# NickDrake117/GNNkeras

Hardware: AMD Instinct MI355X
Metric: node-state updates/s (arcs x iterations / s), forward Loop (higher is better)
Workload: dtype f32; 1 GPU; C4 Erdos-Renyi 1000000 nodes / 10000000 arcs, state_dim=64, max_iteration=50, threshold=0 (k=50), node-focused, average aggregation, BN+Dense(159->64,selu) state net

## Files before the change

gnnkeras_amd/csrc/kernels_train_big.hpp:

```cpp
#pragma once
#include "bf16_split.hpp"
#include <hip/hip_runtime.h>
#include "kernels_general.hpp"
#include "kernel_state_fused4.hpp"
#include <type_traits>
#include "kernel_state_lds.hpp"
#include "kernels_train.hpp"
#include "buffer_ops.hpp"

namespace gnn {

constexpr int TB_STREAM_AUX = 0;
constexpr int TB_RING_AUX = 2;
#define TB_MFMA_DRAIN() asm volatile("s_nop 15\n\ts_nop 3" ::: "memory")
typedef float f32x16 __attribute__((ext_vector_type(16)));
constexpr int TB_WAVES = 8;

template <int LPR, bool HAS_W, bool BUF = false>
__global__ void __launch_bounds__(256, 8)
k_aggregate_stats(const int *gate, int n_dst, const int *__restrict__ rowptr, const int *__restrict__ src,
                  const float *__restrict__ w, const float *__restrict__ row_scale, const float *__restrict__ X, int ldx,
                  float *__restrict__ out, int ldo, float *__restrict__ stat_part, const float *__restrict__ shift) {
    if (gate_closed(gate)) return;
    __shared__ f32x4 red[2][256];
// ... 174 lines not shown
    return activate1<ACT>(v);
}
__device__ __forceinline__ f32x4 fma4(const f32x4 &a, const f32x4 &b, const f32x4 &c) { return __builtin_elementwise_fma(a, b, c); }

__device__ __forceinline__ void split3_store(unsigned short *base, int plane_stride, int idx, float v) {
    const __bf16 vh = (__bf16)v;
    const float r1 = v - (float)vh;
    const __bf16 vm = (__bf16)r1;
    const float r2 = r1 - (float)vm;
    const __bf16 vl = (__bf16)r2;
    base[idx] = __builtin_bit_cast(unsigned short, vh); base[plane_stride + idx] = __builtin_bit_cast(unsigned short, vm);
    base[2 * plane_stride + idx] = __builtin_bit_cast(unsigned short, vl);
}


constexpr int TB_B6_WAVES = 2;
template <int SQ, int ACT, bool ADD>
__device__ __forceinline__ void train_fwd_b6_body(const TrainFwdArgs &a, const int bid, const int nblk) {
    if (gate_closed(a.gate)) return;
    constexpr int XQ = ADD ? 0 : 2;
    constexpr int NCT = SQ, HP = 16 * NCT, NQ = 2 * SQ + XQ, NKB = NQ / 2;
    constexpr int PLANE = NKB * NCT * 64 * 8;
    extern __shared__ __attribute__((aligned(16))) float tb_smem[];
    unsigned short *Wl = reinterpret_cast<unsigned short *>(tb_smem);
    float *bias_l = tb_smem + 3 * PLANE / 2;
    float *red = bias_l + HP;
    float *shift_l = red + TB_WAVES * 2 * HP;
    float *mean_l = shift_l + HP;
    __shared__ int any_s;
    const int tid = threadIdx.x, lane = tid & 63, wave = tid >> 6;
    const int c = lane & 15, g = lane >> 4;
    if (tid == 0) any_s = 0;
    for (int h = tid; h < HP; h += 64 * TB_WAVES) shift_l[h] = (a.stat_shift && h < a.H) ? a.stat_shift[h] : 0.0f;
    for (int k = tid; k < 16 * NQ; k += 64 * TB_WAVES) mean_l[k] = fwd_in_mean(a, SQ, k);
    int *rowtab = reinterpret_cast<int *>(red);
    for (int k = tid; k < 16 * NQ; k += 64 * TB_WAVES) {
        int row = -1;
        if (k < 16 * SQ) row = a.wrow_state + k;
        else if (k < 32 * SQ) row = a.wrow_agg + (k - 16 * SQ);
        else if (!ADD && a.xc) {
            int jj = k - 32 * SQ, beg = 0;
#pragma unroll
            for (int sg = 0; sg < 3; ++sg) {
                if (sg < a.cs.n && jj >= beg && jj < beg + a.cs.width[sg]) row = a.cs.wrow[sg] + (jj - beg);
                if (sg < a.cs.n) beg += a.cs.width[sg];
            }
        }
        rowtab[k] = row;
    }
    __syncthreads();
    {
        const __amdgpu_buffer_rsrc_t r_w = buf_rsrc(a.Wf);
        constexpr int PER = (16 * NQ * HP) / (64 * TB_WAVES), BATCH = PER % 5 == 0 ? 5 : PER % 4 == 0 ? 4 : PER % 3 == 0 ? 3 : PER % 2 == 0 ? 2 : 1;
        static_assert((16 * NQ * HP) % (64 * TB_WAVES) == 0 && (64 * TB_WAVES) % HP == 0 && PER % BATCH == 0, "weight staging: whole batches");
        const int h = tid % HP, k0 = tid / HP;
#pragma unroll 1
        for (int it0 = 0; it0 < PER; it0 += BATCH) {
            float v[BATCH];
#pragma unroll
            for (int u = 0; u < BATCH; ++u) {
                const int k = k0 + (it0 + u) * ((64 * TB_WAVES) / HP), row = rowtab[k];
                v[u] = buf_ld_f32(r_w, (row >= 0 && h < a.H) ? ((unsigned)row * (unsigned)a.H + (unsigned)h) * 4u : BUF_OFF);
            }
#pragma unroll
            for (int u = 0; u < BATCH; ++u) {
                const int k = k0 + (it0 + u) * ((64 * TB_WAVES) / HP);
                const int q = k >> 4, gg = (k >> 2) & 3, e = k & 3;
                split3_store(Wl, PLANE, ((((q >> 1) * NCT + (h >> 4)) * 64 + 16 * gg + (h & 15)) * 8) + 4 * (q & 1) + e, v[u]);
            }
        }
    }
    __syncthreads();
    for (int h = tid; h < HP; h += 64 * TB_WAVES) bias_l[h] = h < a.H ? a.bf[h] : 0.0f;
    __syncthreads();

    const __amdgpu_buffer_rsrc_t r_s = buf_rsrc_n(a.state, (unsigned)a.M * (unsigned)a.ld_state * 4u), r_a = buf_rsrc_n(a.agg, (unsigned)a.M * (unsigned)a.ld_agg * 4u),
                                 r_x = ADD ? buf_rsrc_n(uniform_ptr(a.addend), (unsigned)a.M * (unsigned)a.ld_add * 4u) : buf_rsrc_n(uniform_ptr(a.xc), (unsigned)a.M * 128u),
                                 r_y = buf_rsrc(a.Y);
    const int n_tiles = (a.M + 15) >> 4;
    f32x4 cs1[NCT], cs2[NCT];
#pragma unroll
    for (int ct = 0; ct < NCT; ++ct) { cs1[ct] = (f32x4){0.f, 0.f, 0.f, 0.f}; cs2[ct] = (f32x4){0.f, 0.f, 0.f, 0.f}; }
    int any = 0;
    f32x4 A[NQ];
    f32x4 Cn[ADD ? NCT : 1];
    const unsigned o_s = (unsigned)c * (unsigned)a.ld_state * 4u + 16u * g, o_a = (unsigned)c * (unsigned)a.ld_agg * 4u + 16u * g,
                   o_x = ADD ? (unsigned)c * (unsigned)a.ld_add * 4u + 16u * g : (unsigned)c * 128u + 16u * g;
    auto fetch = [&](int t) {
        const unsigned b_s = 64u * (unsigned)t * (unsigned)a.ld_state + o_s, b_a = 64u * (unsigned)t * (unsigned)a.ld_agg + o_a,
                       b_x = ADD ? 64u * (unsigned)t * (unsigned)a.ld_add + o_x : 2048u * (unsigned)t + o_x;
#pragma unroll
        for (int q = 0; q < SQ; ++q) {
            A[q] = buf_ld_f32x4_aux<TB_STREAM_AUX>(r_s, b_s + 64u * q);
            A[SQ + q] = buf_ld_f32x4_aux<TB_STREAM_AUX>(r_a, b_a + 64u * q);
        }
        if constexpr (ADD) {
#pragma unroll
            for (int ct = 0; ct < NCT; ++ct) Cn[ct] = buf_ld_f32x4_aux<TB_STREAM_AUX>(r_x, b_x + 64u * ct);
        } else {
#pragma unroll
            for (int q = 0; q < XQ; ++q) A[2 * SQ + q] = buf_ld_f32x4_aux<TB_STREAM_AUX>(r_x, b_x + 64u * q);
        }
    };
    const int t_step = nblk * TB_WAVES;
    fetch(bid * TB_WAVES + wave);
    const u32x4 *Wv = reinterpret_cast<const u32x4 *>(Wl) + lane;
    f32x4 vP[NCT];
    int offP = 0; bool inP = false;
#pragma unroll
    for (int ct = 0; ct < NCT; ++ct) vP[ct] = (f32x4){0.f, 0.f, 0.f, 0.f};
#pragma unroll 1
    for (int t = bid * TB_WAVES + wave; t < n_tiles; t += t_step) {
        const int row = 16 * t + c;
        const bool in = row < a.M;
        u32x4 xh[NKB], xm[NKB], xl[NKB];
        f32x4 old[SQ];
#pragma unroll
        for (int kb = 0; kb < NKB; ++kb)
            split3_x8pk(A[2 * kb] - *reinterpret_cast<const f32x4 *>(mean_l + 32 * kb + 4 * g), A[2 * kb + 1] - *reinterpret_cast<const f32x4 *>(mean_l + 32 * kb + 16 + 4 * g),
                        xh[kb], xm[kb], xl[kb]);
#pragma unroll
        for (int q = 0; q < SQ; ++q) old[q] = A[q];
        f32x4 acc[NCT];
#pragma unroll
        for (int ct = 0; ct < NCT; ++ct) {
            acc[ct] = *reinterpret_cast<const f32x4 *>(bias_l + 16 * ct + 4 * g);
            if constexpr (ADD) acc[ct] += Cn[ct];
        }
        __builtin_amdgcn_sched_barrier(0);
        fetch(t + t_step);
#pragma unroll
        for (int ct = 0; ct < NCT; ++ct) {
            const u32x4 bits = {__float_as_uint(vP[ct][0]), __float_as_uint(vP[ct][1]), __float_as_uint(vP[ct][2]), __float_as_uint(vP[ct][3])};
            __builtin_amdgcn_raw_buffer_store_b128(bits, r_y, inP ? offP + (int)((16u * ct + 4u * g) * 4u) : (int)BUF_OFF, 0, 0);
        }
        __builtin_amdgcn_sched_barrier(0);
        constexpr int CTG = NCT < 2 ? NCT : 2, SPK = NCT / CTG, NS = NKB * SPK;
        u32x4 W[2][3][CTG];
        auto load_w = [&](int st, u32x4 (&w)[3][CTG]) {
            const int kb = st / SPK, ct0 = (st % SPK) * CTG;
#pragma unroll
            for (int pl = 0; pl < 3; ++pl)
#pragma unroll
                for (int u = 0; u < CTG; ++u) w[pl][u] = Wv[pl * (PLANE / 8) + (kb * NCT + ct0 + u) * 64];
        };
        load_w(0, W[0]);
#pragma unroll
        for (int st = 0; st < NS; ++st) {
            const int kb = st / SPK, ct0 = (st % SPK) * CTG;
            if (st + 1 < NS) load_w(st + 1, W[(st + 1) & 1]);
            __builtin_amdgcn_sched_barrier(0);
#define B8(v_) __builtin_bit_cast(bf16x8, v_)
#define MF(pl_, x_) _Pragma("unroll") for (int u = 0; u < CTG; ++u) acc[ct0 + u] = __builtin_amdgcn_mfma_f32_16x16x32_bf16(B8(W[st & 1][pl_][u]), B8(x_), acc[ct0 + u], 0, 0, 0)
            MF(2, xh[kb]); MF(0, xl[kb]); MF(1, xm[kb]); MF(1, xh[kb]); MF(0, xm[kb]); MF(0, xh[kb]);
#undef MF
#undef B8
            __builtin_amdgcn_sched_barrier(0);
        }
        asm volatile("s_nop 15\n\ts_nop 3" ::: "memory");
        f32x4 d2v = {0.f, 0.f, 0.f, 0.f}, n2v = {0.f, 0.f, 0.f, 0.f};
        const float mask = in ? 1.0f : 0.0f;
        const f32x4 mask4 = {mask, mask, mask, mask};
#pragma unroll
        for (int ct = 0; ct < NCT; ++ct) {
            f32x4 v = acc[ct];
#pragma unroll
            for (int e = 0; e < 4; ++e) v[e] = activate_b6<ACT>(v[e]);
            vP[ct] = v;
            { const f32x4 dv = (v - *reinterpret_cast<const f32x4 *>(shift_l + 16 * ct + 4 * g)) * mask4; cs1[ct] += dv; cs2[ct] = fma4(dv, dv, cs2[ct]); }
            { const f32x4 dd = v - old[ct]; d2v = fma4(dd, dd, d2v); n2v = fma4(old[ct], old[ct], n2v); }
        }
        float d2 = (d2v[0] + d2v[1]) + (d2v[2] + d2v[3]), n2 = (n2v[0] + n2v[1]) + (n2v[2] + n2v[3]);
        d2 += __shfl_xor(d2, 16, 64); d2 += __shfl_xor(d2, 32, 64);
        n2 += __shfl_xor(n2, 16, 64); n2 += __shfl_xor(n2, 32, 64);
        any |= (in && sqrtf(d2) > a.thr * sqrtf(n2)) ? 1 : 0;
        offP = (int)((unsigned)row * (unsigned)a.ldy * 4u); inP = in;
    }
#pragma unroll
    for (int ct = 0; ct < NCT; ++ct) {
        const u32x4 bits = {__float_as_uint(vP[ct][0]), __float_as_uint(vP[ct][1]), __float_as_uint(vP[ct][2]), __float_as_uint(vP[ct][3])};
        __builtin_amdgcn_raw_buffer_store_b128(bits, r_y, inP ? offP + (int)((16u * ct + 4u * g) * 4u) : (int)BUF_OFF, 0, 0);
    }
    if (a.pred_flag && __any(any) && lane == 0) any_s = 1;
    if (a.stat_part) {
#pragma unroll
        for (int ct = 0; ct < NCT; ++ct)
#pragma unroll
            for (int e = 0; e < 4; ++e) {
                const float s1 = row16_sum_to_lane15(cs1[ct][e]), s2 = row16_sum_to_lane15(cs2[ct][e]);
                if (c == 15) { red[wave * 2 * HP + 16 * ct + 4 * g + e] = s1; red[wave * 2 * HP + HP + 16 * ct + 4 * g + e] = s2; }
            }
    }
    __syncthreads();
    if (a.stat_part && tid < 2 * HP) {
        float tsum = 0.0f;
        for (int w_ = 0; w_ < TB_WAVES; ++w_) tsum += red[w_ * 2 * HP + tid];
        a.stat_part[(size_t)bid * 2 * HP + tid] = tsum;
    }
    if (a.pred_flag && tid == 0) {
        if (any_s) atomicOr(a.pred_flag, 1);
        if (bid == 0 && a.pred_k) *a.pred_k = a.pred_kval;
    }
}

template <int SQ, int ACT, bool ADD = false>
__global__ void __launch_bounds__(64 * TB_WAVES, TB_B6_WAVES) k_train_fwd_b6(TrainFwdArgs a) { train_fwd_b6_body<SQ, ACT, ADD>(a, blockIdx.x, gridDim.x); }
template <int SQ, int ACT, bool ADD>
__global__ void __launch_bounds__(64 * TB_WAVES, TB_B6_WAVES) k_train_fwd_b6_types(TypeLaunch<TrainFwdArgs> m) {
    int bid, nblk;
    const TrainFwdArgs a = select_type(m, bid, nblk);
    train_fwd_b6_body<SQ, ACT, ADD>(a, bid, nblk);
}

template <int SQ, bool ADD = false>
inline size_t train_fwd_b6_lds() {
    constexpr int NQ = 2 * SQ + (ADD ? 0 : 2);
    return (size_t)(3 * (NQ / 2) * SQ * 64 * 8 * 2) + (size_t)(16 * SQ + TB_WAVES * 2 * 16 * SQ + 16 * SQ + 16 * NQ) * sizeof(float);
}

struct TrainBwdArgs {
    int M;
    const float *dZ; int ldz;
    const float *Y; int act;
    const float *W; int ldw;
    int H, S, wrow_state, wrow_agg;
    const float *state; int ld_state; const float *agg; int ld_agg;
    const float *gamma, *mean, *var, *m1, *m2; float eps;
    const float *agg_row_scale;
    float *dx; int ld_dx;
    int defer_state_bn;
};

template <int ACT> __device__ __forceinline__ float activate_grad1(float y) {
    if (ACT == GNN_ACT_RELU) return y > 0.0f ? 1.0f : 0.0f;
    if (ACT == GNN_ACT_SELU) return y > 0.0f ? 1.0507009873554805f : y + 1.0507009873554805f * 1.6732632423543772f;
    if (ACT == GNN_ACT_TANH) return 1.0f - y * y;
    if (ACT == GNN_ACT_SIGMOID) return y * (1.0f - y);
    if (ACT == GNN_ACT_ELU) return y > 0.0f ? 1.0f : y + 1.0f;
    if (ACT == GNN_ACT_SOFTPLUS) return 1.0f - expf(-y);
    return 1.0f;
}

template <int HQ, int ACT>
__device__ __forceinline__ void train_bwd_dx_b6_body(const TrainBwdArgs &a, const int bid, const int nblk) {
    constexpr int NCT = 2 * HQ, HP = 16 * NCT, SQ = HQ, NKB = (HQ + 1) / 2, NW = 4;
    constexpr int PLANE = NKB * NCT * 64 * 8;
    extern __shared__ __attribute__((aligned(16))) float tb_smem[];
    unsigned short *Wl = reinterpret_cast<unsigned short *>(tb_smem);
    float *coef = tb_smem + 3 * PLANE / 2;
    const int tid = threadIdx.x, lane = tid & 63, wave = tid >> 6;
    const int c = lane & 15, g = lane >> 4;
    const int S = a.S;
    {
        const __amdgpu_buffer_rsrc_t r_w = buf_rsrc(a.W);
        constexpr int TOT = 32 * NKB * HP, BATCH = (TOT / (64 * NW)) % 8 == 0 ? 8 : 4;
        static_assert(TOT % (64 * NW * BATCH) == 0, "weight staging: whole batches");
#pragma unroll 1
        for (int i0 = tid; i0 < TOT; i0 += 64 * NW * BATCH) {
            float v[BATCH];
#pragma unroll
            for (int u = 0; u < BATCH; ++u) {
                const int i = i0 + u * 64 * NW, k = i / HP, j = i % HP;
                const int row = j < S ? a.wrow_state + j : a.wrow_agg + (j - S);
                v[u] = buf_ld_f32(r_w, k < a.H ? ((unsigned)row * (unsigned)a.ldw + (unsigned)k) * 4u : BUF_OFF);
            }
#pragma unroll
            for (int u = 0; u < BATCH; ++u) {
                const int i = i0 + u * 64 * NW, k = i / HP, j = i % HP;
                const int q = k >> 4, gg = (k >> 2) & 3, e = k & 3;
                split3_store(Wl, PLANE, ((((q >> 1) * NCT + (j >> 4)) * 64 + 16 * gg + (j & 15)) * 8) + 4 * (q & 1) + e, v[u]);
            }
        }
    }
    for (int j = tid; j < HP; j += 64 * NW) {
        float Ac = 1.0f, Cc = 0.0f, M1 = 0.0f, Mu = 0.0f;
        if (a.gamma) {
            const int k = j < S ? a.wrow_state + j : a.wrow_agg + (j - S);
            const float rstd = 1.0f / sqrtf(a.var[k] + a.eps);
            Ac = a.gamma[k] * rstd; Cc = -Ac * rstd * a.m2[k]; M1 = a.m1[k]; Mu = a.mean[k];
            if (a.defer_state_bn && j < S) { Cc = 0.0f; M1 = 0.0f; Mu = 0.0f; }
        }
        coef[j] = Ac; coef[HP + j] = Cc; coef[2 * HP + j] = M1; coef[3 * HP + j] = Mu;
    }
    __syncthreads();
    const __amdgpu_buffer_rsrc_t r_z = buf_rsrc(a.dZ), r_y = buf_rsrc(a.Y), r_s = buf_rsrc((a.gamma && !a.defer_state_bn) ? a.state : nullptr), r_a = buf_rsrc(a.gamma ? a.agg : nullptr),
                                 r_o = buf_rsrc(a.dx), r_rs = buf_rsrc(a.agg_row_scale);
    const int n_tiles = (a.M + 15) >> 4;
    const int t_step = nblk * NW;
    f32x4 A[HQ], Yv[HQ], X[NCT];
    float rs;
    auto off_row = [&](int t, bool &in_) { const int row_ = 16 * t + c; in_ = t < n_tiles && row_ < a.M; return (unsigned)row_; };
    auto fetch_zy = [&](int t) {
        bool in_; const unsigned r = off_row(t, in_);
#pragma unroll
        for (int q = 0; q < HQ; ++q) {
            A[q] = buf_ld_f32x4_aux<TB_STREAM_AUX>(r_z, in_ ? (r * (unsigned)a.ldz + 16u * q + 4u * g) * 4u : BUF_OFF);
            Yv[q] = buf_ld_f32x4_aux<TB_STREAM_AUX>(r_y, in_ ? (r * (unsigned)a.ldz + 16u * q + 4u * g) * 4u : BUF_OFF);
        }
    };
    auto fetch_x = [&](int t, int ct) {
        bool in_; const unsigned r = off_row(t, in_);
        if (ct < SQ) X[ct] = buf_ld_f32x4_aux<TB_STREAM_AUX>(r_s, in_ ? (r * (unsigned)a.ld_state + 16u * ct + 4u * g) * 4u : BUF_OFF);
        else X[ct] = buf_ld_f32x4_aux<TB_STREAM_AUX>(r_a, in_ ? (r * (unsigned)a.ld_agg + 16u * (ct - SQ) + 4u * g) * 4u : BUF_OFF);
    };
    auto fetch_rs = [&](int t) { bool in_; const unsigned r = off_row(t, in_); rs = buf_ld_f32(r_rs, in_ ? r * 4u : BUF_OFF); };
    {
        const int t0 = bid * NW + wave;
        fetch_zy(t0); fetch_rs(t0);
#pragma unroll
        for (int ct = 0; ct < NCT; ++ct) fetch_x(t0, ct);
    }
    const u32x4 *Wv = reinterpret_cast<const u32x4 *>(Wl) + lane;
    const bool has_rs = a.agg_row_scale != nullptr;
#pragma unroll 1
    for (int t = bid * NW + wave; t < n_tiles; t += t_step) {
        const int row = 16 * t + c;
        const bool in = row < a.M;
        u32x4 xh[NKB], xm[NKB], xl[NKB];
#pragma unroll
        for (int q = 0; q < HQ; ++q)
#pragma unroll
            for (int e = 0; e < 4; ++e) A[q][e] *= activate_grad1<ACT>(Yv[q][e]);
#pragma unroll
        for (int kb = 0; kb < NKB; ++kb) {
            const f32x4 z4 = {0.f, 0.f, 0.f, 0.f};
            split3_x8(A[2 * kb], 2 * kb + 1 < HQ ? A[2 * kb + 1 < HQ ? 2 * kb + 1 : 0] : z4, xh[kb], xm[kb], xl[kb]);
        }
        const float rs_t = has_rs ? rs : 1.0f;
        __builtin_amdgcn_sched_barrier(0);
        fetch_zy(t + t_step); fetch_rs(t + t_step);
        __builtin_amdgcn_sched_barrier(0);
        f32x4 acc[NCT];
#pragma unroll
        for (int ct = 0; ct < NCT; ++ct) acc[ct] = (f32x4){0.f, 0.f, 0.f, 0.f};
        constexpr int CTG = 2, SPK = NCT / CTG, NS = NKB * SPK;
        u32x4 W[2][3][CTG];
        auto load_w = [&](int st, u32x4 (&w)[3][CTG]) {
            const int kb = st / SPK, ct0 = (st % SPK) * CTG;
#pragma unroll
            for (int pl = 0; pl < 3; ++pl)
#pragma unroll
                for (int u = 0; u < CTG; ++u) w[pl][u] = Wv[pl * (PLANE / 8) + (kb * NCT + ct0 + u) * 64];
        };
        load_w(0, W[0]);
#pragma unroll
        for (int st = 0; st < NS; ++st) {
            const int kb = st / SPK, ct0 = (st % SPK) * CTG;
            if (st + 1 < NS) load_w(st + 1, W[(st + 1) & 1]);
            __builtin_amdgcn_sched_barrier(0);
#define B8(v_) __builtin_bit_cast(bf16x8, v_)
#define MF(pl_, x_) _Pragma("unroll") for (int u = 0; u < CTG; ++u) acc[ct0 + u] = __builtin_amdgcn_mfma_f32_16x16x32_bf16(B8(W[st & 1][pl_][u]), B8(x_), acc[ct0 + u], 0, 0, 0)
            MF(2, xh[kb]); MF(0, xl[kb]); MF(1, xm[kb]); MF(1, xh[kb]); MF(0, xm[kb]); MF(0, xh[kb]);
#undef MF
#undef B8
            __builtin_amdgcn_sched_barrier(0);
        }
        asm volatile("s_nop 15\n\ts_nop 3" ::: "memory");
#pragma unroll
        for (int ct = 0; ct < NCT; ++ct) {
            const int j0 = 16 * ct + 4 * g;
            const f32x4 Ac = *reinterpret_cast<const f32x4 *>(coef + j0), Cc = *reinterpret_cast<const f32x4 *>(coef + HP + j0),
                        M1 = *reinterpret_cast<const f32x4 *>(coef + 2 * HP + j0), Mu = *reinterpret_cast<const f32x4 *>(coef + 3 * HP + j0);
            f32x4 v;
#pragma unroll
            for (int e = 0; e < 4; ++e) v[e] = fmaf(Ac[e], acc[ct][e] - M1[e], Cc[e] * (X[ct][e] - Mu[e]));
            if (ct >= SQ) v *= rs_t;
            const u32x4 bits = {__float_as_uint(v[0]), __float_as_uint(v[1]), __float_as_uint(v[2]), __float_as_uint(v[3])};
            __builtin_amdgcn_raw_buffer_store_b128(bits, r_o, in ? (int)(((unsigned)row * (unsigned)a.ld_dx + (unsigned)j0) * 4u) : (int)BUF_OFF, 0, 0);
            fetch_x(t + t_step, ct);
        }
    }
}

template <int HQ, int ACT>
__global__ void __launch_bounds__(256, 2) k_train_bwd_dx_b6(TrainBwdArgs a) { train_bwd_dx_b6_body<HQ, ACT>(a, blockIdx.x, gridDim.x); }
template <int HQ, int ACT>
__global__ void __launch_bounds__(256, 2) k_train_bwd_dx_b6_types(TypeLaunch<TrainBwdArgs> m) {
    int bid, nblk;
    const TrainBwdArgs a = select_type(m, bid, nblk);
    train_bwd_dx_b6_body<HQ, ACT>(a, bid, nblk);
}

template <int HQ>
inline size_t train_bwd_b6_lds() { return (size_t)(3 * ((HQ + 1) / 2) * 2 * HQ * 64 * 8 * 2) + (size_t)(4 * 32 * HQ) * sizeof(float); }

struct TrainWgradArgs {
    int M, rows_per_wg;
    const float *G, *Y; int act;
    const float *state, *agg;
    const float *xc;
    int K, wrow_state, wrow_agg, Kc; ConstCols cs;
    float *part;
    const float *mean;
};

__device__ __forceinline__ int wgrad_wrow(const TrainWgradArgs &a, int S, int kv) {
    if (kv < S) return a.wrow_state + kv;
    if (kv < 2 * S) return a.wrow_agg + (kv - S);
    int jj = kv - 2 * S, b0 = 0, wrow = -1;
#pragma unroll
    for (int sg = 0; sg < 3; ++sg) { if (sg < a.cs.n && jj >= b0 && jj < b0 + a.cs.width[sg]) wrow = a.cs.wrow[sg] + (jj - b0); if (sg < a.cs.n) b0 += a.cs.width[sg]; }
    return wrow;
}

template <int SQ> struct Piece { float v[SQ]; };
template <int SQ> __device__ __forceinline__ Piece<SQ> ld_piece(__amdgpu_buffer_rsrc_t r, unsigned off);
template <> __device__ __forceinline__ Piece<1> ld_piece<1>(__amdgpu_buffer_rsrc_t r, unsigned off) {
    Piece<1> p; p.v[0] = __uint_as_float(__builtin_amdgcn_raw_buffer_load_b32(r, (int)off, 0, 0)); return p; }
template <> __device__ __forceinline__ Piece<2> ld_piece<2>(__amdgpu_buffer_rsrc_t r, unsigned off) {
    typedef unsigned int u32x2 __attribute__((ext_vector_type(2)));
    const u32x2 t = __builtin_amdgcn_raw_buffer_load_b64(r, (int)off, 0, 0);
    Piece<2> p; p.v[0] = __uint_as_float(t[0]); p.v[1] = __uint_as_float(t[1]); return p; }

template <int SQ>
__global__ void __launch_bounds__(256, 2) k_train_wgrad(TrainWgradArgs a) {
    constexpr int S = 16 * SQ, RT = 2 * SQ + 2, KV = 2 * S + 32, PD = 3;
    __shared__ float Ps[KV * S];
    const int tid = threadIdx.x, lane = tid & 63, wave = tid >> 6;
    const int c = lane & 15, g = lane >> 4;
    const int m_beg = blockIdx.x * a.rows_per_wg, m_end = min(a.M, m_beg + a.rows_per_wg);
    const int n_steps = (max(m_end - m_beg, 0) + 15) >> 4;
    const __amdgpu_buffer_rsrc_t r_g = buf_rsrc(a.G), r_y = buf_rsrc(a.Y), r_s = buf_rsrc(a.state), r_a = buf_rsrc(a.agg), r_c = buf_rsrc(a.xc);
    f32x4 acc[RT][SQ];
#pragma unroll
    for (int i = 0; i < RT; ++i)
#pragma unroll
        for (int j = 0; j < SQ; ++j) acc[i][j] = (f32x4){0.f, 0.f, 0.f, 0.f};
    float mu_s[SQ], mu_a[SQ], mu_c[2];
#pragma unroll
    for (int e = 0; e < SQ; ++e) { mu_s[e] = a.mean ? a.mean[a.wrow_state + SQ * c + e] : 0.0f; mu_a[e] = a.mean ? a.mean[a.wrow_agg + SQ * c + e] : 0.0f; }
#pragma unroll
    for (int e = 0; e < 2; ++e) { const int wr = wgrad_wrow(a, S, 2 * S + 2 * c + e); mu_c[e] = (a.mean && wr >= 0) ? a.mean[wr] : 0.0f; }
    struct Step { Piece<SQ> xs, xa, gz, y; Piece<2> xc; };
    Step buf[PD];
    auto fetch = [&](Step &b, int s) {
        const int row = m_beg + 16 * s + 4 * wave + g;
        const bool ok = s < n_steps && row < m_end;
        const unsigned off = ok ? ((unsigned)row * (unsigned)S + (unsigned)(SQ * c)) * 4u : BUF_OFF;
        b.gz = ld_piece<SQ>(r_g, off); b.y = ld_piece<SQ>(r_y, off);
        b.xs = ld_piece<SQ>(r_s, off); b.xa = ld_piece<SQ>(r_a, off);
        b.xc = ld_piece<2>(r_c, ok ? ((unsigned)row * 32u + 2u * c) * 4u : BUF_OFF);
    };
#pragma unroll
    for (int u = 0; u < PD; ++u) fetch(buf[u], u);
#pragma unroll 1
    for (int s0 = 0; s0 < n_steps; s0 += PD) {
#pragma unroll
        for (int u = 0; u < PD; ++u) {
            if (s0 + u < n_steps) {
                Step &b = buf[u];
                float dz[SQ];
#pragma unroll
                for (int j = 0; j < SQ; ++j) dz[j] = b.gz.v[j] * activate_grad_from_output(a.act, b.y.v[j]);
// ... 631 lines not shown
```

gnnkeras_amd/csrc/train_loop.hpp:

```cpp
#pragma once
#include "kernels_train.hpp"
#include "kernels_train_big.hpp"
#include "kernels_train_small.hpp"
#include "kernels_train_labels.hpp"

namespace {

struct NetCtx {
    const gnn_mlp_t *m;
    const gnn_mlp_grads_t *g;
    float *Wt[GNN_MAX_LAYERS];
    float *P, *q, *m1, *m2;
    float *G[2];
    float *hid[GNN_MAX_LAYERS];
    float *dropbuf[GNN_MAX_LAYERS + 1];
};

inline unsigned lowbias32_host(unsigned h) { h ^= h >> 16; h *= 0x7feb352du; h ^= h >> 15; h *= 0x846ca68bu; h ^= h >> 16; return h; }
inline unsigned drop_key(unsigned seed, unsigned net_id, unsigned call, unsigned index) {
    unsigned h = 0x9E3779B9u;
    const unsigned v[4] = {seed, net_id, call, index};
    for (int i = 0; i < 4; ++i) h = lowbias32_host(h ^ v[i]);
    return h;
}
// ... 478 lines not shown
    if (p.with_labels) { segs[n++] = gnn::Seg{p.agg_nodes, nullptr, p.ld_agg_nodes, p.L, col}; col += p.L; }
    if (p.A > 0) { segs[n++] = gnn::Seg{p.agg_arcs, nullptr, p.ld_agg_arcs, p.A, col}; col += p.A; }
    return n;
}

inline bool gather_buf_enabled() { const char *e = getenv("GNN_GATHER_BUF"); return !(e && e[0] == '0'); }
inline bool gather_buf_ok(const gnn_csr_t &c, int ldx) {
    return gather_buf_enabled() && (size_t)c.n_src * (size_t)ldx * 4 < 0xFFFFFFF0ull && (size_t)c.nnz * 4 < 0xFFFFFFF0ull;
}
int launch_aggregate_stats(const int *gate, const gnn_csr_t &c, const float *X, int S, float *out, float *part, float *mean, float *var, const float *shift,
                           hipStream_t st, int *grid_out = nullptr) {
    const int lpr = S / 4, groups = 256 / lpr;
    const int grid = std::min(cdiv(c.n_dst, groups), BIG_AGG_BLOCKS);
#define AGGS_(L, W_, B_) gnn::k_aggregate_stats<L, W_, B_><<<grid, 256, 0, st>>>(gate, c.n_dst, c.rowptr, c.src, c.w, c.row_scale, X, S, out, S, part, shift)
#define AGGS(L) (buf ? (c.w ? AGGS_(L, true, true) : AGGS_(L, false, true)) : (c.w ? AGGS_(L, true, false) : AGGS_(L, false, false)))
    const bool buf = gather_buf_ok(c, S);
    switch (lpr) { case 4: AGGS(4); break; case 8: AGGS(8); break; default: AGGS(16); break; }
#undef AGGS
#undef AGGS_
    LAUNCH_OK();
    if (grid_out) { *grid_out = grid; return 0; }
    gnn::k_stats_finish<<<S, 256, 0, st>>>(gate, part, grid, S, 1.0f / (float)c.n_dst, mean, var, shift);
    LAUNCH_OK();
    return 0;
}

int rows_stats(const int *gate, const float *X, int ld, int F, int M, float *part, hipStream_t st, int *grid_out) {
    const int lpr = F / 4, groups = 256 / lpr;
    const int grid = std::max(1, std::min(cdiv(M, groups * 4), BIG_FWD_BLOCKS));
    switch (lpr) {
        case 4: gnn::k_rows_stats<4><<<grid, 256, 0, st>>>(gate, M, X, ld, part); break;
        case 8: gnn::k_rows_stats<8><<<grid, 256, 0, st>>>(gate, M, X, ld, part); break;
        default: gnn::k_rows_stats<16><<<grid, 256, 0, st>>>(gate, M, X, ld, part); break;
    }
    LAUNCH_OK();
    *grid_out = grid;
    return 0;
}

int line_stats(const float *line, int ld, int M, float *part, const int *width, const int *wrow, int n, float *tpl, int in_dim, hipStream_t st) {
    int grid = 0, c0 = 0;
    TRY(rows_stats(nullptr, line, ld, ld, M, part, st, &grid));
    for (int s = 0; s < n; ++s) {
        gnn::k_stats_finish<<<width[s], 256, 0, st>>>(nullptr, part + c0, grid, ld, 1.0f / (float)M, tpl + wrow[s], tpl + in_dim + wrow[s], line + c0);
        LAUNCH_OK();
        c0 += width[s];
    }
    return 0;
}

template <auto K>
int allow_lds(size_t lds, const char *name) {
    static bool done = false;
    if (!done && hipFuncSetAttribute((const void *)K, hipFuncAttributeMaxDynamicSharedMemorySize, (int)lds) != hipSuccess)
        return fail("%s: cannot raise the dynamic LDS limit", name);
    done = true;
    return 0;
}

template <int SQ, int ACT>
int launch_train_fwd_b6_sa(const gnn::TrainFwdArgs &fa, int grid, hipStream_t st) {
    const size_t lds = gnn::train_fwd_b6_lds<SQ>();
    TRY((allow_lds<gnn::k_train_fwd_b6<SQ, ACT>>(lds, "k_train_fwd_b6")));
    gnn::k_train_fwd_b6<SQ, ACT><<<grid, 64 * gnn::TB_WAVES, lds, st>>>(fa);
    return hipGetLastError() == hipSuccess ? 0 : fail("k_train_fwd_b6 launch failed");
}

template <int SQ>
int launch_train_fwd_b6_s(const gnn::TrainFwdArgs &fa, int grid, hipStream_t st) {
    switch (fa.act) {
        case GNN_ACT_LINEAR: return launch_train_fwd_b6_sa<SQ, GNN_ACT_LINEAR>(fa, grid, st);
        case GNN_ACT_RELU: return launch_train_fwd_b6_sa<SQ, GNN_ACT_RELU>(fa, grid, st);
        case GNN_ACT_SELU: return launch_train_fwd_b6_sa<SQ, GNN_ACT_SELU>(fa, grid, st);
        case GNN_ACT_TANH: return launch_train_fwd_b6_sa<SQ, GNN_ACT_TANH>(fa, grid, st);
        case GNN_ACT_SIGMOID: return launch_train_fwd_b6_sa<SQ, GNN_ACT_SIGMOID>(fa, grid, st);
        case GNN_ACT_ELU: return launch_train_fwd_b6_sa<SQ, GNN_ACT_ELU>(fa, grid, st);
        case GNN_ACT_SOFTPLUS: return launch_train_fwd_b6_sa<SQ, GNN_ACT_SOFTPLUS>(fa, grid, st);
        default: return fail("k_train_fwd_b6: no instance for activation %d", fa.act);
    }
}

int launch_train_fwd(const gnn::TrainFwdArgs &fa, int S, hipStream_t st, int *grid_out) {
    if (fa.H != S) return fail("k_train_fwd_b6: %d units for state width %d", fa.H, S);
    const int n_tiles16 = (fa.M + 15) / 16;
    const int grid = std::max(1, std::min(std::min(device_cus(), BIG_FWD_BLOCKS), cdiv(n_tiles16, gnn::TB_WAVES)));
    *grid_out = grid;
    switch (S) {
        case 16: return launch_train_fwd_b6_s<1>(fa, grid, st);
        case 32: return launch_train_fwd_b6_s<2>(fa, grid, st);
        case 64: return launch_train_fwd_b6_s<4>(fa, grid, st);
        default: return fail("k_train_fwd_b6: no instance for state width %d", S);
    }
}

template <int HQ>
int launch_train_bwd_dx_h(const gnn::TrainBwdArgs &ba, int grid, hipStream_t st) {
    const size_t lds = gnn::train_bwd_b6_lds<HQ>();
    TRY((allow_lds<gnn::k_train_bwd_dx_b6<HQ, GNN_ACT_LINEAR>>(lds, "k_train_bwd_dx_b6")));
    gnn::k_train_bwd_dx_b6<HQ, GNN_ACT_LINEAR><<<grid, 256, lds, st>>>(ba);
    return hipGetLastError() == hipSuccess ? 0 : fail("k_train_bwd_dx_b6 launch failed");
}

int launch_train_bwd_dx(const gnn::TrainBwdArgs &ba, int S, hipStream_t st) {
    if (ba.Y || ba.H != S || ba.S != S || ba.ldz != S) return fail("k_train_bwd_dx_b6: the dZ form of a %d-unit layer only", S);
    const int grid = std::max(1, std::min(2 * device_cus(), cdiv((ba.M + 15) / 16, 4)));
    switch (S) {
        case 16: return launch_train_bwd_dx_h<1>(ba, grid, st);
        case 32: return launch_train_bwd_dx_h<2>(ba, grid, st);
        case 64: return launch_train_bwd_dx_h<4>(ba, grid, st);
        default: return fail("k_train_bwd_dx_b6: no instance for state width %d", S);
    }
}

template <int NB>
int launch_train_wgrad_b6_nb(const gnn::TrainWgradArgs &wa, int grid, hipStream_t st) {
    const size_t lds = gnn::train_wgrad_b6_lds<NB, GNN_ACT_LINEAR>();
    TRY((allow_lds<gnn::k_train_wgrad_b6<NB, GNN_ACT_LINEAR>>(lds, "k_train_wgrad_b6")));
    gnn::k_train_wgrad_b6<NB, GNN_ACT_LINEAR><<<grid, 256, lds, st>>>(wa);
    return hipGetLastError() == hipSuccess ? 0 : fail("k_train_wgrad_b6 launch failed");
}

template <int NB>
int launch_train_wgrad_dx_b6_nb(const gnn::TrainWgradArgs &wa, const gnn::TrainBwdArgs &ba, int grid, hipStream_t st) {
    const size_t lds = gnn::train_wgrad_dx_b6_lds<NB>();
    TRY((allow_lds<gnn::k_train_wgrad_dx_b6<NB>>(lds, "k_train_wgrad_dx_b6")));
    gnn::k_train_wgrad_dx_b6<NB><<<grid, 256, lds, st>>>(wa, ba);
    return hipGetLastError() == hipSuccess ? 0 : fail("k_train_wgrad_dx_b6 launch failed");
}

int launch_train_wgrad(const gnn::TrainWgradArgs &wa, const gnn::TrainBwdArgs *ba, int S, int grid, hipStream_t st) {
    if (wa.Y || wa.act != GNN_ACT_LINEAR) return fail("k_train_wgrad: the dZ form only");
    if (ba) {
        if (ba->gamma || ba->Y || ba->H != S || ba->S != S || ba->ldz != S || ba->ld_state != S || ba->ld_agg != S || ba->M != wa.M || ba->dZ != wa.G ||
            ba->agg != wa.agg || (size_t)wa.rows_per_wg * (size_t)ba->ld_dx * 4 >= 0xFFFFFFF0ull)
            return fail("k_train_wgrad_dx_b6: not for these arguments");
        if (S == 64) return launch_train_wgrad_dx_b6_nb<2>(wa, *ba, grid, st);
        if (S == 32) return launch_train_wgrad_dx_b6_nb<1>(wa, *ba, grid, st);
        return fail("k_train_wgrad_dx_b6: no instance for state width %d", S);
    }
    switch (S) {
        case 16: gnn::k_train_wgrad<1><<<grid, 256, 0, st>>>(wa); LAUNCH_OK(); return 0;
        case 32: return launch_train_wgrad_b6_nb<1>(wa, grid, st);
        case 64: return launch_train_wgrad_b6_nb<2>(wa, grid, st);
        default: return fail("k_train_wgrad: no instance for state width %d", S);
    }
}

template <int LPR, bool HAS_W>
bool launch_aggregate_dz_lw(const gnn_csr_t &c, const float *Xa, int ldx, float *out, int ldo, const float *addend, int ld_add, const gnn::AggDzArgs &z, int act,
                            int grid, hipStream_t st) {
    const bool buf = gather_buf_ok(c, ldx);
#define AGGDZ_(A_, B_) gnn::k_aggregate_dz<LPR, HAS_W, A_, B_><<<grid, 256, 0, st>>>(c.n_dst, c.rowptr, c.src, c.w, c.row_scale, Xa, ldx, out, ldo, addend, ld_add, z)
#define AGGDZ(A_) do { if (buf) AGGDZ_(A_, true); else AGGDZ_(A_, false); } while (0)
    switch (act) {
        case GNN_ACT_LINEAR: AGGDZ(GNN_ACT_LINEAR); return true;
        case GNN_ACT_RELU: AGGDZ(GNN_ACT_RELU); return true;
        case GNN_ACT_SELU: AGGDZ(GNN_ACT_SELU); return true;
        case GNN_ACT_TANH: AGGDZ(GNN_ACT_TANH); return true;
        case GNN_ACT_SIGMOID: AGGDZ(GNN_ACT_SIGMOID); return true;
        case GNN_ACT_ELU: AGGDZ(GNN_ACT_ELU); return true;
        case GNN_ACT_SOFTPLUS: AGGDZ(GNN_ACT_SOFTPLUS); return true;
        default: return false;
    }
#undef AGGDZ
#undef AGGDZ_
}
bool launch_aggregate_dz(const gnn_csr_t &c, const float *Xa, int ldx, float *out, int ldo, const float *addend, int ld_add, const gnn::AggDzArgs &z, int act, int S,
                         hipStream_t st) {
    const int lpr = S / 4, groups = 256 / lpr, grid = std::min(cdiv(c.n_dst, groups), 256 * 16);
    switch (lpr) {
        case 4: return c.w ? launch_aggregate_dz_lw<4, true>(c, Xa, ldx, out, ldo, addend, ld_add, z, act, grid, st) : launch_aggregate_dz_lw<4, false>(c, Xa, ldx, out, ldo, addend, ld_add, z, act, grid, st);
        case 8: return c.w ? launch_aggregate_dz_lw<8, true>(c, Xa, ldx, out, ldo, addend, ld_add, z, act, grid, st) : launch_aggregate_dz_lw<8, false>(c, Xa, ldx, out, ldo, addend, ld_add, z, act, grid, st);
        case 16: return c.w ? launch_aggregate_dz_lw<16, true>(c, Xa, ldx, out, ldo, addend, ld_add, z, act, grid, st) : launch_aggregate_dz_lw<16, false>(c, Xa, ldx, out, ldo, addend, ld_add, z, act, grid, st);
        default: return false;
    }
}

gnn::ConstSegs const_segs_of(const gnn_loop_args_t &a, const TrainPlan &p) {
    gnn::ConstSegs cs{};
    gnn::Seg segs[GNN_MAX_SEGS];
    const int n0 = state_segs(a, p, 0, segs);
    for (int s = 0; s < n0; ++s)
        if (segs[s].ptr != p.states && segs[s].ptr != p.agg) { cs.ptr[cs.n] = segs[s].ptr; cs.ld[cs.n] = segs[s].ld; cs.width[cs.n] = segs[s].width; cs.wrow[cs.n] = segs[s].wrow; ++cs.n; }
    return cs;
}

template <typename Kern, typename Args, typename... Extra>
// ... 834 lines not shown
```

Baseline: 22.12 billion arc-updates/s.

## Double-buffer row tiles two trips ahead in fused train forward and dx kernels

```diff
diff --git a/gnnkeras_amd/csrc/kernels_train_big.hpp b/gnnkeras_amd/csrc/kernels_train_big.hpp
--- a/gnnkeras_amd/csrc/kernels_train_big.hpp
+++ b/gnnkeras_amd/csrc/kernels_train_big.hpp
@@ -280,77 +280,90 @@
 #pragma unroll
     for (int ct = 0; ct < NCT; ++ct) { cs1[ct] = (f32x4){0.f, 0.f, 0.f, 0.f}; cs2[ct] = (f32x4){0.f, 0.f, 0.f, 0.f}; }
     int any = 0;
-    f32x4 A[NQ];
-    f32x4 Cn[ADD ? NCT : 1];
+    typedef f32x4 RowSet[2 * SQ];
+    RowSet A0, A1;
+    f32x4 Xc[ADD ? NCT : XQ];
     const unsigned o_s = (unsigned)c * (unsigned)a.ld_state * 4u + 16u * g, o_a = (unsigned)c * (unsigned)a.ld_agg * 4u + 16u * g,
                    o_x = ADD ? (unsigned)c * (unsigned)a.ld_add * 4u + 16u * g : (unsigned)c * 128u + 16u * g;
-    auto fetch = [&](int t) {
-        const unsigned b_s = 64u * (unsigned)t * (unsigned)a.ld_state + o_s, b_a = 64u * (unsigned)t * (unsigned)a.ld_agg + o_a,
-                       b_x = ADD ? 64u * (unsigned)t * (unsigned)a.ld_add + o_x : 2048u * (unsigned)t + o_x;
-#pragma unroll
-        for (int q = 0; q < SQ; ++q) {
-            A[q] = buf_ld_f32x4_aux<TB_STREAM_AUX>(r_s, b_s + 64u * q);
-            A[SQ + q] = buf_ld_f32x4_aux<TB_STREAM_AUX>(r_a, b_a + 64u * q);
-        }
-        if constexpr (ADD) {
-#pragma unroll
-            for (int ct = 0; ct < NCT; ++ct) Cn[ct] = buf_ld_f32x4_aux<TB_STREAM_AUX>(r_x, b_x + 64u * ct);
-        } else {
-#pragma unroll
-            for (int q = 0; q < XQ; ++q) A[2 * SQ + q] = buf_ld_f32x4_aux<TB_STREAM_AUX>(r_x, b_x + 64u * q);
-        }
-    };
-    const int t_step = nblk * TB_WAVES;
-    fetch(bid * TB_WAVES + wave);
+    auto fetch_chunk = [&](int t, RowSet &A, int q) __attribute__((always_inline)) {
+        if (q < SQ) A[q] = buf_ld_f32x4_aux<TB_STREAM_AUX>(r_s, 64u * (unsigned)t * (unsigned)a.ld_state + o_s + 64u * q);
+        else A[q] = buf_ld_f32x4_aux<TB_STREAM_AUX>(r_a, 64u * (unsigned)t * (unsigned)a.ld_agg + o_a + 64u * (q - SQ));
+    };
+    auto fetch_xc = [&](int t, int j) __attribute__((always_inline)) {
+        Xc[j] = buf_ld_f32x4_aux<TB_STREAM_AUX>(r_x, (ADD ? 64u * (unsigned)t * (unsigned)a.ld_add : 2048u * (unsigned)t) + o_x + 64u * j);
+    };
+    auto store_out = [&](const f32x4 &v, int ct, int row, bool in_) __attribute__((always_inline)) {
+        const u32x4 bits = {__float_as_uint(v[0]), __float_as_uint(v[1]), __float_as_uint(v[2]), __float_as_uint(v[3])};
+        __builtin_amdgcn_raw_buffer_store_b128(bits, r_y, in_ ? (int)((unsigned)row * (unsigned)a.ldy * 4u) + (int)((16u * ct + 4u * g) * 4u) : (int)BUF_OFF, 0, 0);
+    };
+    const int t_step = nblk * TB_WAVES, t_first = __builtin_amdgcn_readfirstlane(bid * TB_WAVES + wave);
     const u32x4 *Wv = reinterpret_cast<const u32x4 *>(Wl) + lane;
-    f32x4 vP[NCT];
-    int offP = 0; bool inP = false;
-#pragma unroll
-    for (int ct = 0; ct < NCT; ++ct) vP[ct] = (f32x4){0.f, 0.f, 0.f, 0.f};
-#pragma unroll 1
-    for (int t = bid * TB_WAVES + wave; t < n_tiles; t += t_step) {
+    auto pad_stores = [&](int n) __attribute__((always_inline)) {
+#pragma unroll
+        for (int i = 0; i < n; ++i) __builtin_amdgcn_raw_buffer_store_b128((u32x4){0u, 0u, 0u, 0u}, r_y, (int)(BUF_OFF - (unsigned)i), 0, 0);
+    };
+    static_assert(NCT <= 16, "pad_stores: offsets BUF_OFF - 15 .. BUF_OFF are out of range of every window");
+    auto request_all = [&](int t, RowSet &A, bool with_xc) __attribute__((always_inline)) {
+        __builtin_amdgcn_sched_barrier(0);
+#pragma unroll
+        for (int q = SQ; q < 2 * SQ; ++q) fetch_chunk(t, A, q);
+        if (with_xc) {
+#pragma unroll
+            for (int j = 0; j < (ADD ? NCT : XQ); ++j) fetch_xc(t_first, j);
+        }
+        pad_stores(NCT);
+#pragma unroll
+        for (int q = 0; q < SQ; ++q) fetch_chunk(t, A, q);
+        __builtin_amdgcn_sched_barrier(0);
+    };
+    request_all(t_first, A0, false);
+    request_all(t_first + t_step, A1, true);
+    auto trip = [&](const int t, RowSet &A) __attribute__((always_inline)) {
         const int row = 16 * t + c;
         const bool in = row < a.M;
-        u32x4 xh[NKB], xm[NKB], xl[NKB];
-        f32x4 old[SQ];
-#pragma unroll
-        for (int kb = 0; kb < NKB; ++kb)
-            split3_x8pk(A[2 * kb] - *reinterpret_cast<const f32x4 *>(mean_l + 32 * kb + 4 * g), A[2 * kb + 1] - *reinterpret_cast<const f32x4 *>(mean_l + 32 * kb + 16 + 4 * g),
-                        xh[kb], xm[kb], xl[kb]);
-#pragma unroll
-        for (int q = 0; q < SQ; ++q) old[q] = A[q];
         f32x4 acc[NCT];
 #pragma unroll
         for (int ct = 0; ct < NCT; ++ct) {
             acc[ct] = *reinterpret_cast<const f32x4 *>(bias_l + 16 * ct + 4 * g);
-            if constexpr (ADD) acc[ct] += Cn[ct];
-        }
-        __builtin_amdgcn_sched_barrier(0);
-        fetch(t + t_step);
-#pragma unroll
-        for (int ct = 0; ct < NCT; ++ct) {
-            const u32x4 bits = {__float_as_uint(vP[ct][0]), __float_as_uint(vP[ct][1]), __float_as_uint(vP[ct][2]), __float_as_uint(vP[ct][3])};
-            __builtin_amdgcn_raw_buffer_store_b128(bits, r_y, inP ? offP + (int)((16u * ct + 4u * g) * 4u) : (int)BUF_OFF, 0, 0);
-        }
+            if constexpr (ADD) { acc[ct] += Xc[ct]; fetch_xc(t + t_step, ct); }
+        }
+        u32x4 xh[2], xm[2], xl[2];
+        auto split = [&](int kb) __attribute__((always_inline)) {
+            const f32x4 m0 = *reinterpret_cast<const f32x4 *>(mean_l + 32 * kb + 4 * g), m1 = *reinterpret_cast<const f32x4 *>(mean_l + 32 * kb + 16 + 4 * g);
+            if (kb < SQ) {
+                split3_x8pk(A[2 * kb] - m0, A[2 * kb + 1] - m1, xh[kb & 1], xm[kb & 1], xl[kb & 1]);
+                if (2 * kb >= SQ) fetch_chunk(t + 2 * t_step, A, 2 * kb);
+                if (2 * kb + 1 >= SQ) fetch_chunk(t + 2 * t_step, A, 2 * kb + 1);
+            } else if constexpr (!ADD) {
+                split3_x8pk(Xc[0] - m0, Xc[1] - m1, xh[kb & 1], xm[kb & 1], xl[kb & 1]);
+                fetch_xc(t + t_step, 0); fetch_xc(t + t_step, 1);
+            }
+        };
+        split(0);
         __builtin_amdgcn_sched_barrier(0);
         constexpr int CTG = NCT < 2 ? NCT : 2, SPK = NCT / CTG, NS = NKB * SPK;
-        u32x4 W[2][3][CTG];
-        auto load_w = [&](int st, u32x4 (&w)[3][CTG]) {
+        u32x4 W0[2][CTG], W1[CTG], W2[CTG];
+        auto load_w = [&](int st, int pl, u32x4 (&w)[CTG]) __attribute__((always_inline)) {
             const int kb = st / SPK, ct0 = (st % SPK) * CTG;
 #pragma unroll
-            for (int pl = 0; pl < 3; ++pl)
-#pragma unroll
-                for (int u = 0; u < CTG; ++u) w[pl][u] = Wv[pl * (PLANE / 8) + (kb * NCT + ct0 + u) * 64];
+            for (int u = 0; u < CTG; ++u) w[u] = Wv[pl * (PLANE / 8) + (kb * NCT + ct0 + u) * 64];
         };
-        load_w(0, W[0]);
+        load_w(0, 2, W2); load_w(0, 0, W0[0]); load_w(0, 1, W1);
 #pragma unroll
         for (int st = 0; st < NS; ++st) {
             const int kb = st / SPK, ct0 = (st % SPK) * CTG;
-            if (st + 1 < NS) load_w(st + 1, W[(st + 1) & 1]);
+            if (st + 1 < NS) load_w(st + 1, 0, W0[(st + 1) & 1]);
+            if (st % SPK == 0 && kb + 1 < NKB) split(kb + 1);
             __builtin_amdgcn_sched_barrier(0);
 #define B8(v_) __builtin_bit_cast(bf16x8, v_)
-#define MF(pl_, x_) _Pragma("unroll") for (int u = 0; u < CTG; ++u) acc[ct0 + u] = __builtin_amdgcn_mfma_f32_16x16x32_bf16(B8(W[st & 1][pl_][u]), B8(x_), acc[ct0 + u], 0, 0, 0)
-            MF(2, xh[kb]); MF(0, xl[kb]); MF(1, xm[kb]); MF(1, xh[kb]); MF(0, xm[kb]); MF(0, xh[kb]);
+#define MF(w_, x_) _Pragma("unroll") for (int u = 0; u < CTG; ++u) acc[ct0 + u] = __builtin_amdgcn_mfma_f32_16x16x32_bf16(B8(w_[u]), B8(x_), acc[ct0 + u], 0, 0, 0)
+            MF(W2, xh[kb & 1]);
+            __builtin_amdgcn_sched_barrier(0);
+            if (st + 1 < NS) load_w(st + 1, 2, W2);
+            MF(W0[st & 1], xl[kb & 1]); MF(W1, xm[kb & 1]); MF(W1, xh[kb & 1]);
+            __builtin_amdgcn_sched_barrier(0);
+            if (st + 1 < NS) load_w(st + 1, 1, W1);
+            MF(W0[st & 1], xm[kb & 1]); MF(W0[st & 1], xh[kb & 1]);
 #undef MF
 #undef B8
             __builtin_amdgcn_sched_barrier(0);
@@ -364,38 +377,44 @@
             f32x4 v = acc[ct];
 #pragma unroll
             for (int e = 0; e < 4; ++e) v[e] = activate_b6<ACT>(v[e]);
-            vP[ct] = v;
+            store_out(v, ct, row, in);
             { const f32x4 dv = (v - *reinterpret_cast<const f32x4 *>(shift_l + 16 * ct + 4 * g)) * mask4; cs1[ct] += dv; cs2[ct] = fma4(dv, dv, cs2[ct]); }
-            { const f32x4 dd = v - old[ct]; d2v = fma4(dd, dd, d2v); n2v = fma4(old[ct], old[ct], n2v); }
+            { const f32x4 dd = v - A[ct]; d2v = fma4(dd, dd, d2v); n2v = fma4(A[ct], A[ct], n2v); }
         }
         float d2 = (d2v[0] + d2v[1]) + (d2v[2] + d2v[3]), n2 = (n2v[0] + n2v[1]) + (n2v[2] + n2v[3]);
         d2 += __shfl_xor(d2, 16, 64); d2 += __shfl_xor(d2, 32, 64);
         n2 += __shfl_xor(n2, 16, 64); n2 += __shfl_xor(n2, 32, 64);
         any |= (in && sqrtf(d2) > a.thr * sqrtf(n2)) ? 1 : 0;
-        offP = (int)((unsigned)row * (unsigned)a.ldy * 4u); inP = in;
-    }
-#pragma unroll
-    for (int ct = 0; ct < NCT; ++ct) {
-        const u32x4 bits = {__float_as_uint(vP[ct][0]), __float_as_uint(vP[ct][1]), __float_as_uint(vP[ct][2]), __float_as_uint(vP[ct][3])};
-        __builtin_amdgcn_raw_buffer_store_b128(bits, r_y, inP ? offP + (int)((16u * ct + 4u * g) * 4u) : (int)BUF_OFF, 0, 0);
-    }
-    if (a.pred_flag && __any(any) && lane == 0) any_s = 1;
+        __builtin_amdgcn_sched_barrier(0);
+#pragma unroll
+        for (int q = 0; q < SQ; ++q) fetch_chunk(t + 2 * t_step, A, q);
+        __builtin_amdgcn_sched_barrier(0);
+    };
+#pragma unroll 1
+    for (int t = t_first; t < n_tiles; t += 2 * t_step) {
+        trip(t, A0);
+        trip(t + t_step, A1);
+    }
+    int tid_e = threadIdx.x;
+    asm volatile("" : "+v"(tid_e));
+    const int lane_e = tid_e & 63, wave_e = tid_e >> 6, c_e = lane_e & 15, g_e = lane_e >> 4;
+    if (a.pred_flag && __any(any) && lane_e == 0) any_s = 1;
     if (a.stat_part) {
 #pragma unroll
         for (int ct = 0; ct < NCT; ++ct)
 #pragma unroll
             for (int e = 0; e < 4; ++e) {
                 const float s1 = row16_sum_to_lane15(cs1[ct][e]), s2 = row16_sum_to_lane15(cs2[ct][e]);
-                if (c == 15) { red[wave * 2 * HP + 16 * ct + 4 * g + e] = s1; red[wave * 2 * HP + HP + 16 * ct + 4 * g + e] = s2; }
+                if (c_e == 15) { red[wave_e * 2 * HP + 16 * ct + 4 * g_e + e] = s1; red[wave_e * 2 * HP + HP + 16 * ct + 4 * g_e + e] = s2; }
             }
     }
     __syncthreads();
-    if (a.stat_part && tid < 2 * HP) {
+    if (a.stat_part && tid_e < 2 * HP) {
         float tsum = 0.0f;
-        for (int w_ = 0; w_ < TB_WAVES; ++w_) tsum += red[w_ * 2 * HP + tid];
-        a.stat_part[(size_t)bid * 2 * HP + tid] = tsum;
-    }
-    if (a.pred_flag && tid == 0) {
+        for (int w_ = 0; w_ < TB_WAVES; ++w_) tsum += red[w_ * 2 * HP + tid_e];
+        a.stat_part[(size_t)bid * 2 * HP + tid_e] = tsum;
+    }
+    if (a.pred_flag && tid_e == 0) {
         if (any_s) atomicOr(a.pred_flag, 1);
         if (bid == 0 && a.pred_k) *a.pred_k = a.pred_kval;
     }
@@ -485,10 +504,13 @@
                                  r_o = buf_rsrc(a.dx), r_rs = buf_rsrc(a.agg_row_scale);
     const int n_tiles = (a.M + 15) >> 4;
     const int t_step = nblk * NW;
-    f32x4 A[HQ], Yv[HQ], X[NCT];
-    float rs;
+    typedef f32x4 ZSet[HQ];
+    typedef f32x4 XSet[NCT];
+    ZSet A0, A1, Y0, Y1;
+    XSet X0, X1;
+    float rs0, rs1;
     auto off_row = [&](int t, bool &in_) { const int row_ = 16 * t + c; in_ = t < n_tiles && row_ < a.M; return (unsigned)row_; };
-    auto fetch_zy = [&](int t) {
+    auto fetch_zy = [&](int t, ZSet &A, ZSet &Yv) __attribute__((always_inline)) {
         bool in_; const unsigned r = off_row(t, in_);
 #pragma unroll
         for (int q = 0; q < HQ; ++q) {
@@ -496,22 +518,29 @@
             Yv[q] = buf_ld_f32x4_aux<TB_STREAM_AUX>(r_y, in_ ? (r * (unsigned)a.ldz + 16u * q + 4u * g) * 4u : BUF_OFF);
         }
     };
-    auto fetch_x = [&](int t, int ct) {
+    auto fetch_x = [&](int t, int ct, XSet &X) __attribute__((always_inline)) {
         bool in_; const unsigned r = off_row(t, in_);
         if (ct < SQ) X[ct] = buf_ld_f32x4_aux<TB_STREAM_AUX>(r_s, in_ ? (r * (unsigned)a.ld_state + 16u * ct + 4u * g) * 4u : BUF_OFF);
         else X[ct] = buf_ld_f32x4_aux<TB_STREAM_AUX>(r_a, in_ ? (r * (unsigned)a.ld_agg + 16u * (ct - SQ) + 4u * g) * 4u : BUF_OFF);
     };
-    auto fetch_rs = [&](int t) { bool in_; const unsigned r = off_row(t, in_); rs = buf_ld_f32(r_rs, in_ ? r * 4u : BUF_OFF); };
-    {
-        const int t0 = bid * NW + wave;
-        fetch_zy(t0); fetch_rs(t0);
-#pragma unroll
-        for (int ct = 0; ct < NCT; ++ct) fetch_x(t0, ct);
-    }
+    auto fetch_rs = [&](int t, float &rs) __attribute__((always_inline)) { bool in_; const unsigned r = off_row(t, in_); rs = buf_ld_f32(r_rs, in_ ? r * 4u : BUF_OFF); };
+    const int t_first = __builtin_amdgcn_readfirstlane(bid * NW + wave);
+    static_assert(NCT <= 16, "offsets BUF_OFF - 15 .. BUF_OFF are out of range of the 4 GiB - 16 window");
+    auto request_all = [&](int t, ZSet &A, ZSet &Yv, XSet &X, float &rs) __attribute__((always_inline)) {
+        __builtin_amdgcn_sched_barrier(0);
+        fetch_zy(t, A, Yv); fetch_rs(t, rs);
+#pragma unroll
+        for (int ct = 0; ct < NCT; ++ct) {
+            __builtin_amdgcn_raw_buffer_store_b128((u32x4){0u, 0u, 0u, 0u}, r_o, (int)(BUF_OFF - (unsigned)ct), 0, 0);
+            fetch_x(t, ct, X);
+        }
+        __builtin_amdgcn_sched_barrier(0);
+    };
+    request_all(t_first, A0, Y0, X0, rs0);
+    request_all(t_first + t_step, A1, Y1, X1, rs1);
     const u32x4 *Wv = reinterpret_cast<const u32x4 *>(Wl) + lane;
     const bool has_rs = a.agg_row_scale != nullptr;
-#pragma unroll 1
-    for (int t = bid * NW + wave; t < n_tiles; t += t_step) {
+    auto trip = [&](const int t, ZSet &A, ZSet &Yv, XSet &X, float &rs) __attribute__((always_inline)) {
         const int row = 16 * t + c;
         const bool in = row < a.M;
         u32x4 xh[NKB], xm[NKB], xl[NKB];
@@ -526,7 +555,7 @@
         }
         const float rs_t = has_rs ? rs : 1.0f;
         __builtin_amdgcn_sched_barrier(0);
-        fetch_zy(t + t_step); fetch_rs(t + t_step);
+        fetch_zy(t + 2 * t_step, A, Yv); fetch_rs(t + 2 * t_step, rs);
         __builtin_amdgcn_sched_barrier(0);
         f32x4 acc[NCT];
 #pragma unroll
@@ -565,8 +594,13 @@
             if (ct >= SQ) v *= rs_t;
             const u32x4 bits = {__float_as_uint(v[0]), __float_as_uint(v[1]), __float_as_uint(v[2]), __float_as_uint(v[3])};
             __builtin_amdgcn_raw_buffer_store_b128(bits, r_o, in ? (int)(((unsigned)row * (unsigned)a.ld_dx + (unsigned)j0) * 4u) : (int)BUF_OFF, 0, 0);
-            fetch_x(t + t_step, ct);
-        }
+            fetch_x(t + 2 * t_step, ct, X);
+        }
+    };
+#pragma unroll 1
+    for (int t = t_first; t < n_tiles; t += 2 * t_step) {
+        trip(t, A0, Y0, X0, rs0);
+        trip(t + t_step, A1, Y1, X1, rs1);
     }
 }
 
diff --git a/gnnkeras_amd/csrc/train_loop.hpp b/gnnkeras_amd/csrc/train_loop.hpp
--- a/gnnkeras_amd/csrc/train_loop.hpp
+++ b/gnnkeras_amd/csrc/train_loop.hpp
@@ -584,6 +584,8 @@
 
 int launch_train_fwd(const gnn::TrainFwdArgs &fa, int S, hipStream_t st, int *grid_out) {
     if (fa.H != S) return fail("k_train_fwd_b6: %d units for state width %d", fa.H, S);
+    const size_t widest = (size_t)std::max(std::max(fa.ld_state, fa.ld_agg), std::max(fa.ldy, fa.xc ? 32 : 0));
+    if ((size_t)fa.M * widest * 4 >= 0xFFFFFFF0ull) return fail("k_train_fwd_b6: %d rows of %zu floats do not fit a 4 GiB window", fa.M, widest);
     const int n_tiles16 = (fa.M + 15) / 16;
     const int grid = std::max(1, std::min(std::min(device_cus(), BIG_FWD_BLOCKS), cdiv(n_tiles16, gnn::TB_WAVES)));
     *grid_out = grid;
@@ -605,6 +607,8 @@
 
 int launch_train_bwd_dx(const gnn::TrainBwdArgs &ba, int S, hipStream_t st) {
     if (ba.Y || ba.H != S || ba.S != S || ba.ldz != S) return fail("k_train_bwd_dx_b6: the dZ form of a %d-unit layer only", S);
+    if ((size_t)ba.M * (size_t)std::max(ba.ld_dx, std::max(ba.ld_state, ba.ld_agg)) * 4 >= 0xFFFFFFF0ull)
+        return fail("k_train_bwd_dx_b6: %d rows of %d floats do not fit a 4 GiB window", ba.M, ba.ld_dx);
     const int grid = std::max(1, std::min(2 * device_cus(), cdiv((ba.M + 15) / 16, 4)));
     switch (S) {
         case 16: return launch_train_bwd_dx_h<1>(ba, grid, st);
```

Result: no change. 22.12 billion arc-updates/s (median of 4 runs) (+0.0%).
